# nv-tlabs/DefTet

Hardware: AMD Instinct MI355X
Metric: M tet-point tests/s (fwd+bwd) at res=70, 100k queries (higher is better)
Workload: dtype f32

## Files before the change

deftet_amd/csrc/point_in_tet.hip:

```cpp
#pragma clang fp contract(off)

#include <stdlib.h>

#include <algorithm>
#include <type_traits>
#include <vector>

#include "common.hpp"

namespace deftet {
namespace pit {

constexpr float kBig = 1048576.0f;
constexpr float kTau = 1.0f / 128.0f;
constexpr float kMargin = 1.0f / 64.0f;
constexpr float kWMin = 9.3132257e-10f;
constexpr int kMiss = 0x7F7F7F7F;
constexpr int kMaxG = 112;
constexpr int kMaxBins = 15 * 1024;
constexpr int kHitOverflow = -2;

constexpr int kHitPad = 64;
__host__ __device__ inline int hit_pad(int B) { return (B + kHitPad - 1) / kHitPad * kHitPad; }
__host__ __device__ inline size_t hit_cnt_off(int B, int T) { return (size_t)B * T * 2; }
// ... 1225 lines not shown
            if (__builtin_amdgcn_ballot_w64(cnew > cap) != 0ull) {
                if (cnew > cap) {
                    int *resb = result + (size_t)b * Q;
                    if (hcnt > 0) atomicMin(&resb[h0], t);
                    if (hcnt > 1) atomicMin(&resb[h1], t);
                    if (hcnt > 2) atomicMin(&resb[h2], t);
                    if (hcnt > 3) atomicMin(&resb[h3], t);
                    on_full();
                }
            }
#pragma unroll
            for (int k = 0; k < PIT_BATCH; ++k) {
                const int qi = __float_as_int(q[k].w);
                h3 = sel(acc[k], h2, h3);
                h2 = sel(acc[k], h1, h2);
                h1 = sel(acc[k], h0, h1);
                h0 = sel(acc[k], qi, h0);
                hcnt += sel(acc[k], 1, 0);
            }
            c += PIT_BATCH;
        }
    }
    PHASE_MARK(1);
    if (npend > 0) {
        const typename TS::Ref tv = ts.at(b, T, t);
        atomicAdd(&counters[gridDim.y * 4 + b * 4 + 1], npend);
        if (npend > 2) {
            exact_rescan<TS>(tv, t, tb, sq, result + (size_t)b * Q, G, Gx, cx0, cx1, cy0, cy1, cz0, cz1, m, counters, gridDim.y, b, hits, spill, (size_t)b * T + t);
            irregular_tail<TS>(tet, t, b, T, Q, pts, counters, irregQ, result);
            return;
        }
        for (int k = 0; k < npend; ++k) {
            const float4 q = sq[k == 0 ? pend0 : pend1];
            if (exact_accept<TS>(tv, q.x, q.y, q.z) > 0.f) {
                const int qi = __float_as_int(q.w);
                atomicMin(&result[(size_t)b * Q + qi], t);
                if (hcnt >= cap) {
                    int *resb = result + (size_t)b * Q;
                    atomicMin(&resb[h0], t); atomicMin(&resb[h1], t);
                    if (hcnt > 2) atomicMin(&resb[h2], t);
                    if (hcnt > 3) atomicMin(&resb[h3], t);
                    on_full();
                }
                h3 = h2; h2 = h1; h1 = h0; h0 = qi;
                ++hcnt;
            }
        }
    }
    int *resb = uniform_ptr(result + (size_t)b * Q);
    if (hcnt > 0) atomic_smin_off(resb, (unsigned)h0 * 4u, t);
    if (hcnt > 1) atomic_smin_off(resb, (unsigned)h1 * 4u, t);
    if (hcnt > 2) atomic_smin_off(resb, (unsigned)h2 * 4u, t);
    if (hcnt > 3) atomic_smin_off(resb, (unsigned)h3 * 4u, t);
    if (full == 1 && hcnt > cap) full = 2;
    if (full == 2) note_overflow(counters, gridDim.y, b, t);
    if (hits) {
        if (full == 0) {
            const lanemask_t sp = mask_of(hcnt > 2);
            store_b64_off(uniform_ptr(hits + (size_t)b * T), (unsigned)t * 8u, sel(sp, h0 | kHitSpilled, h0), h1);
            if (hcnt > 2) store_b128_off(uniform_ptr(spill + (size_t)b * T), (unsigned)t * 16u, h2, h3, -1, -1);
        } else if (full == 1) {
            int *sp = reinterpret_cast<int *>(spill + (size_t)b * T + t) + scnt;
            if (hcnt > 0) sp[0] = h0;
            if (hcnt > 1) sp[1] = h1;
            if (hcnt > 2) sp[2] = h2;
            if (hcnt > 3) sp[3] = h3;
        } else {
            store_b64_off(uniform_ptr(hits + (size_t)b * T), (unsigned)t * 8u, -1, kHitOverflow);
        }
    }
    irregular_tail<TS>(tet, t, b, T, Q, pts, counters, irregQ, result);
    PHASE_MARK(2);
}

constexpr int kWvRows = 192;
#ifndef PIT_WVCAP
#define PIT_WVCAP 96
#endif
constexpr int kWvCap = PIT_WVCAP;
constexpr int kWvSlots = 6;
#ifndef PIT_WG
#define PIT_WG 128
#endif
constexpr int kWvThreads = PIT_WG;
static_assert(kWvThreads % 64 == 0 && kWvThreads >= 64 && kWvThreads <= 256, "whole waves");
static_assert(kWvRows % 64 == 0 && kWvSlots >= 4 && kWvSlots <= 8, "whole waves of row ids; the records hold four + four");
#ifndef PIT_WVCAP_PAIR
#define PIT_WVCAP_PAIR 128
#endif
constexpr int kWvCapPair = PIT_WVCAP_PAIR, kWvRowsPair = 256;
#ifndef PIT_DBG_WALK
#define PIT_DBG_WALK 1
#endif
#ifndef PIT_DBG_PEND
#define PIT_DBG_PEND 1
#endif
#ifndef PIT_STOP
#define PIT_STOP 0
#endif
#define PIT_KEEP(x) asm volatile("" ::"v"(x))
#ifndef PIT_PROBE_SKIP
#define PIT_PROBE_SKIP 0
#endif
#ifndef PIT_PROBE_PREFILL
#define PIT_PROBE_PREFILL 0
#endif
#ifndef PIT_PIN_SHAPES
#define PIT_PIN_SHAPES 0
#endif
#ifndef PIT_PROBE_SCATTER
#define PIT_PROBE_SCATTER 0
#endif
#ifndef PIT_WAVES_PAIR
#define PIT_WAVES_PAIR 5
#endif
#ifndef PIT_TOLX
#define PIT_TOLX 2
#endif
#ifndef PIT_MINGROUP
#define PIT_MINGROUP 4
#endif
constexpr int kWvMinGroup = PIT_MINGROUP;
#ifndef PIT_ZREACH
#define PIT_ZREACH 24
#endif
constexpr int kWvZReach = PIT_ZREACH;
constexpr float kRelScale = 2.86102294921875e-06f;
constexpr float kTauSlim = kTau * (1.0f + 1.0f / 128.0f);
#ifndef PIT_WAVES2
#define PIT_WAVES2 7
#endif
template <int CAP, int ROWS>
struct __attribute__((aligned(16))) WaveStageT {
    typedef typename std::conditional<(ROWS <= 254), unsigned char, unsigned short>::type marker_t;
    float4 q[CAP];
    int delta[ROWS];
    unsigned short rowBase[ROWS + 4];
    marker_t marker[CAP];
};

template <int CTRL, int ROW_MASK>
__device__ __forceinline__ int dpp0(int v)
{
    return __builtin_amdgcn_update_dpp(0, v, CTRL, ROW_MASK, 0xf, true);
}
__device__ __forceinline__ int wave_scan_add(int x)
{
    x += dpp0<0x111, 0xf>(x); x += dpp0<0x112, 0xf>(x); x += dpp0<0x114, 0xf>(x); x += dpp0<0x118, 0xf>(x);
    x += dpp0<0x142, 0xa>(x); x += dpp0<0x143, 0xc>(x);
    return x;
}
__device__ __forceinline__ int wave_scan_max(int x)
{
    x = max(x, dpp0<0x111, 0xf>(x)); x = max(x, dpp0<0x112, 0xf>(x)); x = max(x, dpp0<0x114, 0xf>(x)); x = max(x, dpp0<0x118, 0xf>(x));
    x = max(x, dpp0<0x142, 0xa>(x)); x = max(x, dpp0<0x143, 0xc>(x));
    return x;
}
typedef unsigned short u16x2 __attribute__((ext_vector_type(2)));
__device__ __forceinline__ unsigned pk_max(unsigned a, unsigned b)
{
    const u16x2 r = __builtin_elementwise_max(__builtin_bit_cast(u16x2, a), __builtin_bit_cast(u16x2, b));
    return __builtin_bit_cast(unsigned, r);
}
__device__ __forceinline__ unsigned wave_pk_max(unsigned v)
{
    v = pk_max(v, (unsigned)dpp0<0x111, 0xf>((int)v)); v = pk_max(v, (unsigned)dpp0<0x112, 0xf>((int)v));
    v = pk_max(v, (unsigned)dpp0<0x114, 0xf>((int)v)); v = pk_max(v, (unsigned)dpp0<0x118, 0xf>((int)v));
    v = pk_max(v, (unsigned)dpp0<0x142, 0xf>((int)v)); v = pk_max(v, (unsigned)dpp0<0x143, 0xf>((int)v));
    return (unsigned)__builtin_amdgcn_readlane((int)v, 63);
}
__device__ __forceinline__ void wave_sync()
{
    __builtin_amdgcn_fence(__ATOMIC_ACQ_REL, "wavefront");
    __builtin_amdgcn_wave_barrier();
}
__device__ __forceinline__ void atomic_smin_off_nh(int *base, unsigned byte_off, int v)
{
    asm volatile("global_atomic_smin %0, %1, %2" ::"v"(byte_off), "v"(v), "s"(base) : "memory");
}

__device__ __forceinline__ float sel(lanemask_t m, float if_set, float if_clear)
{
    return __int_as_float(sel(m, __float_as_int(if_set), __float_as_int(if_clear)));
}
__device__ __forceinline__ void cross_fma(float ax, float ay, float az, float bx, float by, float bz, float *n)
{
    n[0] = fmaf(ay, bz, -(az * by));
    n[1] = fmaf(az, bx, -(ax * bz));
    n[2] = fmaf(ax, by, -(ay * bx));
}

template <class TS>
__device__ __noinline__ void irregular_tet_slow(typename TS::Arg tet, int t, int b, int T, int Q, const float *__restrict__ pts,
                                                int *counters, int *irregT, const int *__restrict__ irregQ, int *result, int2 *hits)
{
    const int k = atomicAdd(&counters[b * 4 + 0], 1);
    irregT[(size_t)b * T + k] = t;
    if (hits) hits[(size_t)b * T + t] = make_int2(-1, kHitOverflow);
    if (counters[b * 4 + 1] > 0) irregular_tail_slow<TS>(tet, t, b, T, Q, pts, counters, irregQ, result);
}

__device__ __forceinline__ void tet_cell_box(const float *__restrict__ tv, const Grid &g, int G, int Gx, CellBox &cb, float &mrg)
{
    float blo[3], bhi[3], wk[3];
#pragma unroll
    for (int k = 0; k < 3; ++k) {
        blo[k] = fminf(fminf(tv[k], tv[3 + k]), fminf(tv[6 + k], tv[9 + k]));
        bhi[k] = fmaxf(fmaxf(tv[k], tv[3 + k]), fmaxf(tv[6 + k], tv[9 + k]));
        wk[k] = bhi[k] - blo[k];
    }
    const float w = fmaxf(fmaxf(wk[0], wk[1]), wk[2]);
    mrg = w * kMargin;
    cb.cx0 = cell_of(blo[0] - mrg, g.o[0], g.inv[0], Gx); cb.cx1 = cell_of(bhi[0] + mrg, g.o[0], g.inv[0], Gx);
    cb.cy0 = cell_of(blo[1] - mrg, g.o[1], g.inv[1], G); cb.cy1 = cell_of(bhi[1] + mrg, g.o[1], g.inv[1], G);
    cb.cz0 = cell_of(blo[2] - mrg, g.o[2], g.inv[2], G); cb.cz1 = cell_of(bhi[2] + mrg, g.o[2], g.inv[2], G);
}

template <class TS>
__device__ __noinline__ int exact_rescan_slots(typename TS::RefArg tv, int t, const int *__restrict__ tb, const float4 *__restrict__ sq,
                                               int *res, const float *__restrict__ gp, int G, int Gx, int *slotCol)
{
    float vv[12];
    TS::get(tv, vv);
    Planes P;
    make_planes(vv, P);
    const Grid g = load_grid(gp);
    CellBox cb;
    float m;
    tet_cell_box(vv, g, G, Gx, cb, m);
    float elo[3], ehi[3];
#pragma unroll
    for (int k = 0; k < 3; ++k) {
        elo[k] = fminf(fminf(vv[k], vv[3 + k]), fminf(vv[6 + k], vv[9 + k])) - m;
        ehi[k] = fmaxf(fmaxf(vv[k], vv[3 + k]), fmaxf(vv[6 + k], vv[9 + k])) + m;
    }
    const int Gp = table_pitch(G);
    int hcnt = 0;
    for (int cz = cb.cz0; cz <= cb.cz1; ++cz)
        for (int cy = cb.cy0; cy <= cb.cy1; ++cy) {
            const int s = tb[table_off(cz, cb.cx0, cy, Gx, Gp)], e = tb[table_off(cz, cb.cx1 + 1, cy, Gx, Gp)];
            for (int j = s; j < e; ++j) {
                const float4 q = sq[j];
                if (q.x >= elo[0] && q.x <= ehi[0] && q.y >= elo[1] && q.y <= ehi[1] && q.z >= elo[2] && q.z <= ehi[2] &&
                    accept(P, q.x, q.y, q.z)) {
                    const int qi = __float_as_int(q.w);
                    atomicMin(&res[qi], t);
                    slotCol[min(hcnt, kWvSlots) * kWvThreads] = qi;
                    ++hcnt;
                }
            }
        }
    return hcnt;
}

__device__ __forceinline__ float triple(const float *a, const float *b, const float *c)
{
    float x0 = b[1] * c[2] - b[2] * c[1];
    float x1 = b[2] * c[0] - b[0] * c[2];
    float x2 = b[0] * c[1] - b[1] * c[0];
    return (a[0] * x0 + a[1] * x1) + a[2] * x2;
}
__device__ __forceinline__ float4 bary_weights(const float4 t0, const float4 t1, const float4 t2, float px, float py, float pz)
{
    const float A[3] = {t0.x, t0.y, t0.z}, Bv[3] = {t0.w, t1.x, t1.y}, Cv[3] = {t1.z, t1.w, t2.x}, D[3] = {t2.y, t2.z, t2.w};
    const float pp[3] = {px, py, pz};
    float vap[3], vbp[3], vab[3], vac[3], vad[3], vbc[3], vbd[3];
#pragma unroll
    for (int k = 0; k < 3; ++k) {
        vap[k] = pp[k] - A[k]; vbp[k] = pp[k] - Bv[k];
        vab[k] = Bv[k] - A[k]; vac[k] = Cv[k] - A[k]; vad[k] = D[k] - A[k];
        vbc[k] = Cv[k] - Bv[k]; vbd[k] = D[k] - Bv[k];
    }
    const float v6 = 1.0f / triple(vab, vac, vad);
    float4 wq;
    wq.x = triple(vbp, vbd, vbc) * v6;
    wq.y = triple(vap, vac, vad) * v6;
    wq.z = triple(vap, vad, vab) * v6;
    wq.w = triple(vap, vab, vac) * v6;
    return wq;
}

template <class TS, bool ORD, int NT>
__device__ __forceinline__ void tet_scan_wave_body(typename TS::Arg tet, int T, int Q,
                                                  const float *__restrict__ gparam, int G, int Gx, const int *__restrict__ table,
                                                  long long cellStride, const float4 *__restrict__ sortedQ, int *result, int *counters,
                                                  int *irregT, int2 *hits, const float *__restrict__ pts,
                                                  const int *__restrict__ irregQ, int *ucount, int hpad, int4 *spill,
                                                  const int *__restrict__ order)
{
    constexpr int CAP = NT == 1 ? kWvCap : kWvCapPair, ROWS = NT == 1 ? kWvRows : kWvRowsPair;
    typedef WaveStageT<CAP, ROWS> Stage;
    __shared__ Stage s_w[kWvThreads / 64];
    __shared__ int s_hit[NT][kWvSlots + 2][kWvThreads];
#if PIT_PIN_SHAPES
    const int pinL = blockIdx.y * gridDim.x + blockIdx.x, pinB = gridDim.y;
#define PIT_BLK_B (pinL % pinB)
#define PIT_BLK_X (pinL / pinB)
#else
#define PIT_BLK_B blockIdx.y
#define PIT_BLK_X blockIdx.x
#endif
    if (ucount && PIT_BLK_X == 0 && __builtin_amdgcn_readfirstlane(threadIdx.x) == 0) {
        ucount[PIT_BLK_B] = 0;
        ucount[hpad + PIT_BLK_B] = 0;
        ucount[2 * hpad + PIT_BLK_B] = 0;
    }
    const int b = PIT_BLK_B, tid = threadIdx.x, lane = tid & 63;
    const TS ts(tet);
    Stage &W = s_w[tid >> 6];
    const int nblk = gridDim.x;
#if PIT_PIN_SHAPES
    const int vb = PIT_BLK_X;
#else
    const int per = (nblk + 7) >> 3;
    const int vb = (blockIdx.x & 7) * per + (blockIdx.x >> 3);
#endif
#undef PIT_BLK_B
#undef PIT_BLK_X
    const int t = vb * blockDim.x + tid;
    const bool valid = vb < nblk && t < (T + NT - 1) / NT;
    if (__builtin_amdgcn_ballot_w64(valid) == 0ull) return;
    auto tet_id = [&](int k) -> int {
        const int p = min(NT * t + k, T - 1);
        return ORD ? order[p] : p;
    };
    auto tet_exists = [&](int k) -> bool { return valid && (NT == 1 || NT * t + k < T); };
    PHASE_DECL;
    SPAN_MARK(0);
    const Grid g = load_grid(gparam + b * kGridWords);
    Filter F[NT];
    float eabsMax[NT], mrg[NT], wk[NT][3];
    bool regular[NT], works[NT];
    int cx0 = 0x7FFF, cx1 = 0, cy0 = 0x7FFF, cy1 = 0, cz0 = 0x7FFF, cz1 = 0;
#pragma unroll
    for (int k = 0; k < NT; ++k) {
        float v[12];
        TS::template get4<PIT_SCAN_TET_NT != 0>(ts.at(b, T, tet_id(k)), v);
        float mN[4][3], det;
        {
            const float e1x = v[3] - v[0], e1y = v[4] - v[1], e1z = v[5] - v[2];
            const float e2x = v[6] - v[0], e2y = v[7] - v[1], e2z = v[8] - v[2];
            const float e3x = v[9] - v[0], e3y = v[10] - v[1], e3z = v[11] - v[2];
            cross_fma(e1x, e1y, e1z, e2x, e2y, e2z, mN[0]);
            cross_fma(e3x, e3y, e3z, e1x, e1y, e1z, mN[1]);
            cross_fma(e2x, e2y, e2z, e3x, e3y, e3z, mN[2]);
#pragma unroll
            for (int j = 0; j < 3; ++j) mN[3][j] = -((mN[0][j] + mN[1][j]) + mN[2][j]);
            det = fmaf(mN[0][0], e3x, fmaf(mN[0][1], e3y, mN[0][2] * e3z));
        }
        float blo[3], bhi[3], mx[3];
#pragma unroll
        for (int j = 0; j < 3; ++j) {
            blo[j] = fminf(fminf(v[j], v[3 + j]), fminf(v[6 + j], v[9 + j]));
            bhi[j] = fmaxf(fmaxf(v[j], v[3 + j]), fmaxf(v[6 + j], v[9 + j]));
            wk[k][j] = bhi[j] - blo[j];
            mx[j] = fmaxf(fabsf(blo[j]), fabsf(bhi[j]));
        }
        const float w = fmaxf(fmaxf(wk[k][0], wk[k][1]), wk[k][2]);
        regular[k] = fmaxf(fmaxf(mx[0], mx[1]), mx[2]) <= kBig && w >= kWMin && fabsf(det) >= kTauSlim * ((w * w) * w);
        mrg[k] = w * kMargin;
        float elo[3], ehi[3];
#pragma unroll
        for (int j = 0; j < 3; ++j) {
            elo[j] = blo[j] - mrg[k];
            ehi[j] = bhi[j] + mrg[k];
        }
        const bool ingrid = !(ehi[0] < g.lo[0] || elo[0] > g.hi[0] || ehi[1] < g.lo[1] || elo[1] > g.hi[1] || ehi[2] < g.lo[2] || elo[2] > g.hi[2]);
        {
            const int ax0 = cell_of(elo[0], g.o[0], g.inv[0], Gx), ax1 = cell_of(ehi[0], g.o[0], g.inv[0], Gx);
            const int ay0 = cell_of(elo[1], g.o[1], g.inv[1], G), ay1 = cell_of(ehi[1], g.o[1], g.inv[1], G);
            const int az0 = cell_of(elo[2], g.o[2], g.inv[2], G), az1 = cell_of(ehi[2], g.o[2], g.inv[2], G);
            regular[k] = regular[k] && !(ingrid && wide_tet(ax0, ax1, ay0, ay1, az0, az1, g));
            works[k] = tet_exists(k) && regular[k] && ingrid;
            if (NT == 1) {
                cx0 = ax0; cx1 = ax1; cy0 = ay0; cy1 = ay1; cz0 = az0; cz1 = az1;
            } else if (works[k]) {
                cx0 = min(cx0, ax0); cx1 = max(cx1, ax1); cy0 = min(cy0, ay0); cy1 = max(cy1, ay1); cz0 = min(cz0, az0); cz1 = max(cz1, az1);
            }
        }
        const float sigma = det > 0.f ? 1.0f : -1.0f;
        float S[3];
#pragma unroll
        for (int j = 0; j < 3; ++j) S[j] = fmaf(mx[j], 2.0f * kErrScale, g.pe[j]);
        eabsMax[k] = 0.f;
#pragma unroll
        for (int i = 0; i < 4; ++i) {
            const float n0 = mN[i][0], n1 = mN[i][1], n2 = mN[i][2];
            const float *a = i < 3 ? v : v + 3;
            const float c = fmaf(n0, a[0], fmaf(n1, a[1], n2 * a[2]));
            const float E = fmaf(fabsf(n0), S[0], fmaf(fabsf(n1), S[1], fabsf(n2) * S[2]));
            F[k].N[i][0] = sigma * n0; F[k].N[i][1] = sigma * n1; F[k].N[i][2] = sigma * n2;
            F[k].C[i] = fmaf(-sigma, c, -E);
            eabsMax[k] = fmaxf(eabsMax[k], E);
        }
    }
    bool work = works[0];
#pragma unroll
    for (int k = 1; k < NT; ++k) work = work || works[k];
    if (PIT_STOP == 1) {
#pragma unroll
        for (int i = 0; i < 4; ++i) { PIT_KEEP(F[0].N[i][0]); PIT_KEEP(F[0].N[i][1]); PIT_KEEP(F[0].N[i][2]); PIT_KEEP(F[0].C[i]); }
        PIT_KEEP(eabsMax[0]); PIT_KEEP(mrg[0]); PIT_KEEP(wk[0][0]); PIT_KEEP(wk[0][1]); PIT_KEEP(wk[0][2]);
        PIT_KEEP(cx0); PIT_KEEP(cx1); PIT_KEEP(cy0); PIT_KEEP(cy1); PIT_KEEP(cz0); PIT_KEEP(cz1); PIT_KEEP((int)work);
        return;
    }
    const int Gp = table_pitch(G);
    const int *tb = table + (size_t)b * cellStride;
    const float4 *sq = sortedQ + (size_t)b * Q;
    int gx0[2], gx1[2], gy0[2], gz0[2], gny[2], gnz[2], gsh[2];
    int gid = -1;
    int ncx = cx1 - cx0 + 1, ncy = cy1 - cy0 + 1;
    int rowsTot = 0, rowOff1 = 0, slabsTot = 0;
    {
        lanemask_t rem = __builtin_amdgcn_ballot_w64(work);
        int ng = 0;
#pragma unroll
        for (int p = 0; p < 2; ++p) {
            gx0[p] = gx1[p] = gy0[p] = gz0[p] = 0;
            gny[p] = gnz[p] = gsh[p] = 0;
        }
#pragma unroll
        for (int p = 0; p < 3; ++p) {
            if (ng == 2 || __popcll(rem) < kWvMinGroup) break;
            const int pl = __ffsll((long long)rem) - 1;
            const int px0 = __builtin_amdgcn_readlane(cx0, pl), px1 = __builtin_amdgcn_readlane(cx1, pl);
            const int py0 = __builtin_amdgcn_readlane(cy0, pl), py1 = __builtin_amdgcn_readlane(cy1, pl);
            const int pz0 = __builtin_amdgcn_readlane(cz0, pl);
            const bool in = ((rem >> lane) & 1ull) != 0ull && (unsigned)(cx0 - px0 + PIT_TOLX) <= 2u * PIT_TOLX && (unsigned)(cx1 - px1 + PIT_TOLX) <= 2u * PIT_TOLX &&
                            (unsigned)(cy0 - py0 + 1) <= 2u && (unsigned)(cy1 - py1 + 1) <= 2u && (unsigned)(cz0 - pz0 + kWvZReach) <= 2u * kWvZReach;
            const lanemask_t gm = __builtin_amdgcn_ballot_w64(in);
            rem &= ~gm;
            if (__popcll(gm) < kWvMinGroup) { REASON_COUNT(2, gm); continue; }
            const unsigned ax = wave_pk_max(in ? ((unsigned)cx1 | ((0xFFFFu - (unsigned)cx0) << 16)) : 0u);
            const unsigned ay = wave_pk_max(in ? ((unsigned)cy1 | ((0xFFFFu - (unsigned)cy0) << 16)) : 0u);
            const unsigned az = wave_pk_max(in ? ((unsigned)cz1 | ((0xFFFFu - (unsigned)cz0) << 16)) : 0u);
            const int ux0 = (int)(0xFFFFu - (ax >> 16)), uy0 = (int)(0xFFFFu - (ay >> 16)), uz0 = (int)(0xFFFFu - (az >> 16));
            const int ny = (int)(ay & 0xFFFFu) - uy0 + 1, nz = (int)(az & 0xFFFFu) - uz0 + 1;
            const int sh = ny <= 1 ? 0 : 32 - __builtin_clz((unsigned)(ny - 1));
            if (sh > 2 || slabsTot + nz > 64 || rowsTot + (nz << sh) > ROWS) {
                REASON_COUNT(sh > 2 ? 3 : slabsTot + nz > 64 ? 4 : 5, gm);
                continue;
            }
            const bool second = ng != 0;
            gx0[0] = second ? gx0[0] : ux0; gx1[0] = second ? gx1[0] : (int)(ax & 0xFFFFu); gy0[0] = second ? gy0[0] : uy0; gz0[0] = second ? gz0[0] : uz0;
            gny[0] = second ? gny[0] : ny; gnz[0] = second ? gnz[0] : nz; gsh[0] = second ? gsh[0] : sh;
            gx0[1] = second ? ux0 : 0; gx1[1] = second ? (int)(ax & 0xFFFFu) : 0; gy0[1] = second ? uy0 : 0; gz0[1] = second ? uz0 : 0;
            gny[1] = second ? ny : 0; gnz[1] = second ? nz : 0; gsh[1] = second ? sh : 0;
            if (second) rowOff1 = rowsTot;
            rowsTot += nz << sh;
            slabsTot += nz;
            if (in) { gid = ng; ncx = (int)(ax & 0xFFFFu) - ux0 + 1; ncy = ny; }
            ++ng;
        }
        REASON_COUNT(6, rem);
    }
#pragma unroll
    for (int k = 0; k < NT; ++k) {
        const float R0 = fmaf(2.0f, mrg[k], wk[k][0]) + (float)(ncx + 1) * g.cs[0];
        const float R1 = fmaf(2.0f, mrg[k], wk[k][1]) + (float)(ncy + 1) * g.cs[1];
        const float R2 = fmaf(2.0f, mrg[k], wk[k][2]) + (float)(cz1 - cz0 + 2) * g.cs[2];
        const float erel = fmaf(kRelScale, fmaf(wk[k][1] * wk[k][2], R0, fmaf(wk[k][0] * wk[k][2], R1, (wk[k][0] * wk[k][1]) * R2)), kErrAbs);
#pragma unroll
        for (int i = 0; i < 4; ++i) F[k].C[i] -= erel;
        F[k].twoEmax = 2.0f * (eabsMax[k] + erel);
        if (NT > 1 && !works[k]) {
#pragma unroll
            for (int i = 0; i < 4; ++i) { F[k].N[i][0] = F[k].N[i][1] = F[k].N[i][2] = 0.f; F[k].C[i] = -INFINITY; }
            F[k].twoEmax = 0.f;
        }
    }
    if (PIT_STOP == 2) {
#pragma unroll
        for (int i = 0; i < 4; ++i) { PIT_KEEP(F[0].N[i][0]); PIT_KEEP(F[0].N[i][1]); PIT_KEEP(F[0].N[i][2]); PIT_KEEP(F[0].C[i]); }
        PIT_KEEP(F[0].twoEmax); PIT_KEEP(gid); PIT_KEEP(rowsTot); PIT_KEEP(rowOff1); PIT_KEEP(cz0); PIT_KEEP(cz1);
        return;
    }
    PHASE_MARK(0);
    int *resb = uniform_ptr(result + (size_t)b * Q);
    asm volatile("s_nop 4" ::: "memory");
    unsigned slot0[NT], slotEnd[NT], slotA[NT];
#pragma unroll
    for (int k = 0; k < NT; ++k) {
        slot0[k] = (unsigned)(k * (kWvSlots + 2) * kWvThreads + tid) * 4u;
        slotEnd[k] = slot0[k] + (unsigned)(kWvSlots + 1) * (unsigned)(kWvThreads * 4);
        slotA[k] = slot0[k];
    }
    int pend0 = -1, pend1 = -1, npend = 0;
    typedef float f32x2 __attribute__((ext_vector_type(2)));
    f32x2 Px01[NT], Py01[NT], Pz01[NT], Pc01[NT], Px23[NT], Py23[NT], Pz23[NT], Pc23[NT];
#pragma unroll
    for (int k = 0; k < NT; ++k) {
        Px01[k] = f32x2{F[k].N[0][0], F[k].N[1][0]}; Py01[k] = f32x2{F[k].N[0][1], F[k].N[1][1]};
        Pz01[k] = f32x2{F[k].N[0][2], F[k].N[1][2]}; Pc01[k] = f32x2{F[k].C[0], F[k].C[1]};
        Px23[k] = f32x2{F[k].N[2][0], F[k].N[3][0]}; Py23[k] = f32x2{F[k].N[2][1], F[k].N[3][1]};
        Pz23[k] = f32x2{F[k].N[2][2], F[k].N[3][2]}; Pc23[k] = f32x2{F[k].C[2], F[k].C[3]};
    }
    auto test = [&](const float4 q) {
        const f32x2 qx = {q.x, q.x}, qy = {q.y, q.y}, qz = {q.z, q.z};
        const int qi = __float_as_int(q.w);
        float av[NT];
#pragma unroll
        for (int k = 0; k < NT; ++k) {
            const f32x2 A01 = __builtin_elementwise_fma(Px01[k], qx, __builtin_elementwise_fma(Py01[k], qy, __builtin_elementwise_fma(Pz01[k], qz, Pc01[k])));
            const f32x2 A23 = __builtin_elementwise_fma(Px23[k], qx, __builtin_elementwise_fma(Py23[k], qy, __builtin_elementwise_fma(Pz23[k], qz, Pc23[k])));
            av[k] = fminf(fminf(A01.x, A01.y), fminf(A23.x, A23.y));
        }
#pragma unroll
        for (int k = 0; k < NT; ++k)
            if (av[k] > F[k].twoEmax) {
                *reinterpret_cast<int *>(reinterpret_cast<char *>(&s_hit[0][0][0]) + slotA[k]) = qi;
                slotA[k] = min(slotA[k] + (unsigned)(kWvThreads * 4), slotEnd[k]);
            }
        bool band = fabsf(av[0]) <= F[0].twoEmax;
#pragma unroll
        for (int k = 1; k < NT; ++k) band = band || fabsf(av[k]) <= F[k].twoEmax;
        if (__builtin_amdgcn_ballot_w64(band) != 0ull) {
            asm volatile("" ::: "memory");
#pragma unroll
            for (int k = 0; k < NT; ++k) {
                const bool bk = fabsf(av[k]) <= F[k].twoEmax;
                pend1 = bk ? pend0 : pend1;
                pend0 = bk ? (qi | (k << 30)) : pend0;
                npend = bk ? npend + 1 : npend;
            }
        }
    };
    if (rowsTot > 0) {
        const int nzA = gnz[0];
        const bool second = lane >= nzA, slabLane = lane < slabsTot;
        const lanemask_t m2 = mask_of(second);
        const int zl = sel(m2, lane - nzA, lane), sh = sel(m2, gsh[1], gsh[0]), ny = sel(m2, gny[1], gny[0]);
        const int rowId0 = sel(m2, rowOff1, 0) + (zl << sh);
        int a[4], len[4];
        {
            const unsigned zrow = (unsigned)(sel(m2, gz0[1], gz0[0]) + (slabLane ? zl : 0)) * (unsigned)(Gx + 1);
            const unsigned la = ((zrow + (unsigned)sel(m2, gx0[1], gx0[0])) * (unsigned)Gp + (unsigned)sel(m2, gy0[1], gy0[0])) * 4u;
            const unsigned le = ((zrow + (unsigned)sel(m2, gx1[1], gx1[0]) + 1u) * (unsigned)Gp + (unsigned)sel(m2, gy0[1], gy0[0])) * 4u;
            const int4u a0 = ld_off_u4(tb, la), e0 = ld_off_u4(tb, le);
            a[0] = a0.x; a[1] = a0.y; a[2] = a0.z; a[3] = a0.w;
            len[0] = e0.x - a0.x; len[1] = e0.y - a0.y; len[2] = e0.z - a0.z; len[3] = e0.w - a0.w;
        }
        int pre[5];
        pre[0] = 0;
        int lmax = 0;
#pragma unroll
        for (int y = 0; y < 4; ++y) {
            len[y] = sel(mask_of(slabLane && y < ny), len[y], 0);
            pre[y + 1] = pre[y] + len[y];
            lmax = max(lmax, len[y]);
        }
        const int incl = wave_scan_add(pre[4]);
        const int lb = incl - pre[4];
        const int N = __builtin_amdgcn_readlane(incl, 63);
        const int Rtot = rowsTot;
        const bool fitsRows = __builtin_amdgcn_ballot_w64(lmax > CAP) == 0ull && N < 65536;
        if (slabLane) {
#pragma unroll
            for (int y = 0; y < 4; ++y)
                if (y < (1 << sh)) {
                    W.rowBase[rowId0 + y] = (unsigned short)(lb + pre[y]);
                    W.delta[rowId0 + y] = a[y] - (lb + pre[y]);
                }
        }
        if (lane == 0) W.rowBase[Rtot] = (unsigned short)N;
        wave_sync();
        if (PIT_STOP == 3) {
#pragma unroll
            for (int i = 0; i < 4; ++i) { PIT_KEEP(F[0].N[i][0]); PIT_KEEP(F[0].N[i][1]); PIT_KEEP(F[0].N[i][2]); PIT_KEEP(F[0].C[i]); }
            PIT_KEEP(F[0].twoEmax); PIT_KEEP(gid); PIT_KEEP(N); PIT_KEEP(lb); PIT_KEEP(cz0); PIT_KEEP(cz1);
            return;
        }
        PHASE_MARK(4);
        const lanemask_t mine2 = mask_of(gid == 1);
        const int rowOff = sel(mine2, rowOff1, 0), gz = sel(mine2, gz0[1], gz0[0]), gs = sel(mine2, gsh[1], gsh[0]);
        int rn = rowOff + ((cz0 - gz) << gs);
        const int re = rowOff + ((cz1 + 1 - gz) << gs);
        if (!fitsRows) { REASON_COUNT(7, __builtin_amdgcn_ballot_w64(gid >= 0)); gid = -1; }
        int r0 = fitsRows ? 0 : Rtot;
#pragma unroll 1
        while (r0 < Rtot) {
            const int B0 = __builtin_amdgcn_readfirstlane(W.rowBase[r0]);
            int r1 = Rtot;
            if (N - B0 > CAP) {
                r1 = r0;
#pragma unroll 1
                for (int j = 0; j < ROWS / 64; ++j) {
                    const int rc = r0 + 1 + lane + 64 * j;
                    const int cnt = rc <= Rtot ? W.rowBase[rc] - B0 : 0x7FFFFFFF;
                    const lanemask_t fits = __builtin_amdgcn_ballot_w64(cnt <= CAP);
                    if (fits == ~0ull) { r1 += 64; continue; }
                    r1 += __ffsll((long long)~fits) - 1;
                    break;
                }
            }
            const int Nc = __builtin_amdgcn_readfirstlane(W.rowBase[r1]) - B0;
            for (int i = lane; i < Nc; i += 64) W.marker[i] = 0;
            wave_sync();
            if (slabLane) {
                int p0 = W.rowBase[rowId0];
#pragma unroll
                for (int y = 0; y < 4; ++y) {
                    if (y < (1 << sh)) {
                        const int r = rowId0 + y, p1 = W.rowBase[r + 1];
                        if (p1 > p0 && r >= r0 && r < r1) W.marker[p0 - B0] = (typename Stage::marker_t)(r + 1);
                        p0 = p1;
                    }
                }
            }
            wave_sync();
            int carry = 0;
#pragma unroll
            for (int j = 0; j < (CAP + 63) / 64; ++j)
                if (j * 64 < Nc) {
                    const int i = lane + 64 * j;
                    const int own = max(wave_scan_max(i < Nc ? W.marker[i] : 0), carry);
                    carry = __builtin_amdgcn_readlane(own, 63);
                    if (i < Nc) W.q[i] = ld_off<float4>(sq, (unsigned)(B0 + i + W.delta[own - 1]) * 16u);
                }
            wave_sync();
            PHASE_MARK(5);
            PHASE_COUNT(7, Nc);
            PHASE_COUNT(15, 1);
            const int lo = max(rn, r0), hi = min(re, r1);
            if (PIT_STOP != 4 && gid >= 0 && lo < hi) {
                unsigned c = (unsigned)(W.rowBase[lo] - B0) * 16u;
                const unsigned e = (unsigned)(W.rowBase[hi] - B0) * 16u;
                PHASE_COUNT(13, (e - c) >> 4);
                rn = hi;
                const char *qb0 = reinterpret_cast<const char *>(&W.q[0]);
                if (c < e) {
                    float4 qa = *reinterpret_cast<const float4 *>(qb0 + c);
                    for (;;) {
                        const float4 qb = *reinterpret_cast<const float4 *>(qb0 + c + 16);
                        test(qa);
                        c += 16;
                        if (c >= e) break;
                        qa = *reinterpret_cast<const float4 *>(qb0 + c + 16);
                        test(qb);
                        c += 16;
                        if (c >= e) break;
                    }
                }
            }
            wave_sync();
            PHASE_MARK(6);
            r0 = r1;
        }
    }
    PHASE_COUNT(14, __popcll(__builtin_amdgcn_ballot_w64(work && gid < 0)));
    PHASE_MARK(1);
    if (PIT_DBG_WALK && work && gid < 0) {
        CellBox cb;
        {
            cb.cx0 = cb.cy0 = cb.cz0 = 0x7FFF;
            cb.cx1 = cb.cy1 = cb.cz1 = 0;
#pragma unroll
            for (int k = 0; k < NT; ++k) {
                if (NT > 1 && !works[k]) continue;
                float tv[12], mrg2;
                TS::get(ts.at(b, T, tet_id(k)), tv);
                CellBox c1;
                tet_cell_box(tv, g, G, Gx, c1, mrg2);
                cb.cx0 = min(cb.cx0, c1.cx0); cb.cx1 = max(cb.cx1, c1.cx1); cb.cy0 = min(cb.cy0, c1.cy0); cb.cy1 = max(cb.cy1, c1.cy1);
                cb.cz0 = min(cb.cz0, c1.cz0); cb.cz1 = max(cb.cz1, c1.cz1);
            }
        }
        const int cx0 = cb.cx0, cx1 = cb.cx1, cy0 = cb.cy0, cy1 = cb.cy1, cz1 = cb.cz1, czn = cb.cz0;
        const int ny = cy1 - cy0 + 1;
        const unsigned lineB = (unsigned)Gp * 4u;
        const unsigned slabB = (unsigned)(Gx + 1) * lineB;
        const unsigned dxB = (unsigned)(cx1 + 1 - cx0) * lineB;
        unsigned offS = ((unsigned)czn * (unsigned)(Gx + 1) + (unsigned)cx0) * lineB + (unsigned)cy0 * 4u;
        int cz = czn, yoff = 0;
        int4u nS = ld_off_u4(tb, offS), nE = ld_off_u4(tb, offS + dxB);
        bool haveNext = true;
        int c = 0, P1 = 0, P2 = 0, P3 = 0, P4 = 0, o0 = 0, o1 = 0, o2 = 0, o3 = 0;
        while (c < P4 || haveNext) {
            if (c >= P4) {
                const int rem = ny - yoff;
                const int n0 = nE.x - nS.x;
                const int n1 = rem > 1 ? nE.y - nS.y : 0;
                const int n2 = rem > 2 ? nE.z - nS.z : 0;
                const int n3 = rem > 3 ? nE.w - nS.w : 0;
                P1 = n0; P2 = P1 + n1; P3 = P2 + n2; P4 = P3 + n3;
                o0 = nS.x; o1 = nS.y - P1; o2 = nS.z - P2; o3 = nS.w - P3;
                c = 0;
                asm volatile("" : "+v"(P1), "+v"(P2), "+v"(P3), "+v"(P4), "+v"(o0), "+v"(o1), "+v"(o2), "+v"(o3));
                const bool wrap = rem <= 4;
                offS += wrap ? slabB - (unsigned)yoff * 4u : 16u;
                yoff = wrap ? 0 : yoff + 4;
                cz += wrap ? 1 : 0;
                haveNext = cz <= cz1;
                if (haveNext) {
                    nS = ld_off_u4(tb, offS);
                    nE = ld_off_u4(tb, offS + dxB);
                }
            }
            if (c < P4) {
                const int jq = c + (c < P1 ? o0 : c < P2 ? o1 : c < P3 ? o2 : o3);
                test(ld_off<float4>(sq, (unsigned)jq * 16u));
                ++c;
            }
        }
    }
    PHASE_MARK(2);
    if (PIT_STOP == 5) { PIT_KEEP(slotA[0]); PIT_KEEP(pend0); PIT_KEEP(pend1); PIT_KEEP(npend); return; }
    if (!valid) return;
    int hcnt[NT];
#pragma unroll
    for (int k = 0; k < NT; ++k) hcnt[k] = (int)((slotA[k] - slot0[k]) / (unsigned)(kWvThreads * 4));
    if (PIT_DBG_PEND && npend > 0) {
        atomicAdd(&counters[gridDim.y * 4 + b * 4 + 1], npend);
        if (npend > 2) {
#pragma unroll
            for (int k = 0; k < NT; ++k)
                if (works[k]) {
                    const int te = tet_id(k);
                    hcnt[k] = exact_rescan_slots<TS>(ts.at(b, T, te), te, tb, sq, result + (size_t)b * Q, gparam + b * kGridWords, G, Gx,
                                                 &s_hit[k][0][tid]);
                }
        } else {
            for (int j = 0; j < npend; ++j) {
                const int pq = j == 0 ? pend0 : pend1;
                const int k = NT == 1 ? 0 : (pq >> 30) & 1, qi = pq & 0x3FFFFFFF;
                const int te = tet_id(k);
                const float *pp = pts + ((size_t)b * Q + qi) * 3;
                if (exact_accept<TS>(ts.at(b, T, te), pp[0], pp[1], pp[2]) > 0.f) {
                    atomicMin(&result[(size_t)b * Q + qi], te);
                    if (NT == 1 || k == 0) { s_hit[0][min(hcnt[0], kWvSlots)][tid] = qi; ++hcnt[0]; }
                    else { s_hit[NT - 1][min(hcnt[NT - 1], kWvSlots)][tid] = qi; ++hcnt[NT - 1]; }
                }
            }
        }
    }
#pragma unroll
    for (int k = 0; k < NT; ++k) {
        if (NT > 1 && !tet_exists(k)) continue;
        int te = tet_id(k);
        asm volatile("" : "+v"(te));
        if (!regular[k]) {
            irregular_tet_slow<TS>(tet, te, b, T, Q, pts, counters, irregT, irregQ, result, hits);
            continue;
        }
        int hc = hcnt[k];
        if (hc > kWvSlots) {
            const typename TS::Ref tv = ts.at(b, T, te);
            hc = exact_rescan_slots<TS>(tv, te, tb, sq, result + (size_t)b * Q, gparam + b * kGridWords, G, Gx, &s_hit[k][0][tid]);
        }
#pragma unroll 1
        for (int i = 0; i < kWvSlots; ++i) {
            if (__builtin_amdgcn_ballot_w64(hc > i) == 0ull) break;
#if PIT_PROBE_SCATTER == 0
            if (hc > i && !(PIT_PROBE_SKIP & 1)) atomic_smin_off_nh(resb, (unsigned)s_hit[k][i][tid] * 4u, te);
#else
            if (hc > i && spill) {
                const int qi = s_hit[k][i][tid];
                char *pb = reinterpret_cast<char *>(spill);
                const size_t nq = (size_t)gridDim.y * Q, iq = (size_t)b * Q + qi;
                bool win = true;
                if (PIT_PROBE_SCATTER == 1) atomic_smin_off_nh(resb, (unsigned)qi * 4u, te);
                else win = atomicMin(&result[iq], te) > te;
                if (win && PIT_PROBE_SCATTER == 3) {
                    float4 s0, s1, s2;
                    TS::get3(ts.at(b, T, te), s0, s1, s2);
                    const float *pp = pts + iq * 3;
                    *reinterpret_cast<float4 *>(pb + iq * 16) = bary_weights(s0, s1, s2, pp[0], pp[1], pp[2]);
                    *reinterpret_cast<float *>(pb + nq * 16 + iq * 4) = (float)te;
                    *reinterpret_cast<float *>(pb + nq * 20 + iq * 4) = (float)qi;
                } else if (win) {
                    *reinterpret_cast<float4 *>(pb + iq * 16) = make_float4((float)te, (float)qi, 0.25f, 0.5f);
                    *reinterpret_cast<float *>(pb + nq * 16 + iq * 4) = (float)te;
                    *reinterpret_cast<float *>(pb + nq * 20 + iq * 4) = (float)qi;
                }
            }
#endif
        }
        if (hits) {
            int h[kRecSlots + kSpillSlots];
#pragma unroll
            for (int i = 0; i < kRecSlots + kSpillSlots; ++i) h[i] = -1;
#pragma unroll
            for (int i = 0; i < kRecSlots; ++i)
                if (i < hc) h[i] = s_hit[k][i][tid];
            const bool spilled = hc > kRecSlots && hc <= kWvSlots && spill != nullptr && PIT_PROBE_SCATTER == 0;
            const bool over = hc > kRecSlots && !spilled;
            if (spilled) {
#pragma unroll
                for (int i = kRecSlots; i < kWvSlots; ++i)
                    if (i < hc) h[i] = s_hit[k][i][tid];
                spill[(size_t)b * T + te] = make_int4(h[2], h[3], h[4], h[5]);
                h[0] |= kHitSpilled;
            }
            if (over) note_overflow(counters, gridDim.y, b, te);
            if (!(PIT_PROBE_SKIP & 2)) store_rec(hits + (size_t)b * T + te, over ? make_int2(-1, kHitOverflow) : make_int2(h[0], h[1]));
        }
        irregular_tail<TS>(tet, te, b, T, Q, pts, counters, irregQ, result);
    }
    PHASE_MARK(3);
    SPAN_MARK(1);
// ... 1298 lines not shown
```

Measured before the change: 1.102 billion.

## Pack per-tet setup into f32x2/u16x2 SIMD ops and simplify wave grouping

Vectorizes the per-tet filter setup (margins, cell coordinates, plane constants, sigma scaling) with packed f32x2 math, and replaces cell_of with a fmed3 clamp. Wave grouping now compares packed 16-bit x/y ranges and gets group bounds through ballots over tolerance offsets, which removes two packed max reductions. Slab address setup precomputes per-group bases, and the chunk loop tracks B0 incrementally with an unrolled marker clear. The goal is to cut VALU and cross-lane instruction count in setup. It carries a risk of subtle equivalence issues, for example the clamp semantics of cell_of versus fmed3.

Result: no change. 1.101 billion, median of 2 (-0.1%).

```diff
diff --git a/deftet_amd/csrc/point_in_tet.hip b/deftet_amd/csrc/point_in_tet.hip
--- a/deftet_amd/csrc/point_in_tet.hip
+++ b/deftet_amd/csrc/point_in_tet.hip
@@ -1401,9 +1401,10 @@
 }
 __device__ __forceinline__ int wave_scan_max(int x)
 {
-    x = max(x, dpp0<0x111, 0xf>(x)); x = max(x, dpp0<0x112, 0xf>(x)); x = max(x, dpp0<0x114, 0xf>(x)); x = max(x, dpp0<0x118, 0xf>(x));
-    x = max(x, dpp0<0x142, 0xa>(x)); x = max(x, dpp0<0x143, 0xc>(x));
-    return x;
+    unsigned u = (unsigned)x;
+    u = max(u, (unsigned)dpp0<0x111, 0xf>((int)u)); u = max(u, (unsigned)dpp0<0x112, 0xf>((int)u)); u = max(u, (unsigned)dpp0<0x114, 0xf>((int)u));
+    u = max(u, (unsigned)dpp0<0x118, 0xf>((int)u)); u = max(u, (unsigned)dpp0<0x142, 0xa>((int)u)); u = max(u, (unsigned)dpp0<0x143, 0xc>((int)u));
+    return (int)u;
 }
 typedef unsigned short u16x2 __attribute__((ext_vector_type(2)));
 __device__ __forceinline__ unsigned pk_max(unsigned a, unsigned b)
@@ -1577,6 +1578,7 @@
     PHASE_DECL;
     SPAN_MARK(0);
     const Grid g = load_grid(gparam + b * kGridWords);
+    typedef float f32x2 __attribute__((ext_vector_type(2)));
     Filter F[NT];
     float eabsMax[NT], mrg[NT], wk[NT][3];
     bool regular[NT], works[NT];
@@ -1609,16 +1611,20 @@
         regular[k] = fmaxf(fmaxf(mx[0], mx[1]), mx[2]) <= kBig && w >= kWMin && fabsf(det) >= kTauSlim * ((w * w) * w);
         mrg[k] = w * kMargin;
         float elo[3], ehi[3];
+        f32x2 cf[3];
 #pragma unroll
         for (int j = 0; j < 3; ++j) {
-            elo[j] = blo[j] - mrg[k];
-            ehi[j] = bhi[j] + mrg[k];
+            const f32x2 e = f32x2{blo[j], bhi[j]} + f32x2{-mrg[k], mrg[k]};
+            elo[j] = e.x;
+            ehi[j] = e.y;
+            cf[j] = (e - f32x2{g.o[j], g.o[j]}) * f32x2{g.inv[j], g.inv[j]};
         }
         const bool ingrid = !(ehi[0] < g.lo[0] || elo[0] > g.hi[0] || ehi[1] < g.lo[1] || elo[1] > g.hi[1] || ehi[2] < g.lo[2] || elo[2] > g.hi[2]);
         {
-            const int ax0 = cell_of(elo[0], g.o[0], g.inv[0], Gx), ax1 = cell_of(ehi[0], g.o[0], g.inv[0], Gx);
-            const int ay0 = cell_of(elo[1], g.o[1], g.inv[1], G), ay1 = cell_of(ehi[1], g.o[1], g.inv[1], G);
-            const int az0 = cell_of(elo[2], g.o[2], g.inv[2], G), az1 = cell_of(ehi[2], g.o[2], g.inv[2], G);
+            auto cell = [](float f, int n) -> int { return (int)__builtin_amdgcn_fmed3f(f, 0.f, (float)(n - 1)); };
+            const int ax0 = cell(cf[0].x, Gx), ax1 = cell(cf[0].y, Gx);
+            const int ay0 = cell(cf[1].x, G), ay1 = cell(cf[1].y, G);
+            const int az0 = cell(cf[2].x, G), az1 = cell(cf[2].y, G);
             regular[k] = regular[k] && !(ingrid && wide_tet(ax0, ax1, ay0, ay1, az0, az1, g));
             works[k] = tet_exists(k) && regular[k] && ingrid;
             if (NT == 1) {
@@ -1632,15 +1638,33 @@
 #pragma unroll
         for (int j = 0; j < 3; ++j) S[j] = fmaf(mx[j], 2.0f * kErrScale, g.pe[j]);
         eabsMax[k] = 0.f;
+        float cc[4], EE[4];
 #pragma unroll
         for (int i = 0; i < 4; ++i) {
             const float n0 = mN[i][0], n1 = mN[i][1], n2 = mN[i][2];
             const float *a = i < 3 ? v : v + 3;
-            const float c = fmaf(n0, a[0], fmaf(n1, a[1], n2 * a[2]));
-            const float E = fmaf(fabsf(n0), S[0], fmaf(fabsf(n1), S[1], fabsf(n2) * S[2]));
-            F[k].N[i][0] = sigma * n0; F[k].N[i][1] = sigma * n1; F[k].N[i][2] = sigma * n2;
-            F[k].C[i] = fmaf(-sigma, c, -E);
-            eabsMax[k] = fmaxf(eabsMax[k], E);
+            if (i >= 2) cc[i] = fmaf(n0, a[0], fmaf(n1, a[1], n2 * a[2]));
+            EE[i] = fmaf(fabsf(n0), S[0], fmaf(fabsf(n1), S[1], fabsf(n2) * S[2]));
+            eabsMax[k] = fmaxf(eabsMax[k], EE[i]);
+        }
+        {
+            const f32x2 c01 = __builtin_elementwise_fma(f32x2{mN[0][0], mN[1][0]}, f32x2{v[0], v[0]},
+                              __builtin_elementwise_fma(f32x2{mN[0][1], mN[1][1]}, f32x2{v[1], v[1]}, f32x2{mN[0][2], mN[1][2]} * f32x2{v[2], v[2]}));
+            cc[0] = c01.x;
+            cc[1] = c01.y;
+        }
+        const f32x2 sg = {sigma, sigma};
+#pragma unroll
+        for (int h = 0; h < 4; h += 2) {
+#pragma unroll
+            for (int j = 0; j < 3; ++j) {
+                const f32x2 n = sg * f32x2{mN[h][j], mN[h + 1][j]};
+                F[k].N[h][j] = n.x;
+                F[k].N[h + 1][j] = n.y;
+            }
+            const f32x2 C = __builtin_elementwise_fma(-sg, f32x2{cc[h], cc[h + 1]}, -f32x2{EE[h], EE[h + 1]});
+            F[k].C[h] = C.x;
+            F[k].C[h + 1] = C.y;
         }
     }
     bool work = works[0];
@@ -1663,6 +1687,8 @@
     {
         lanemask_t rem = __builtin_amdgcn_ballot_w64(work);
         int ng = 0;
+        const u16x2 xx = {(unsigned short)cx0, (unsigned short)cx1}, yy = {(unsigned short)cy0, (unsigned short)cy1};
+        const unsigned zz = (unsigned)cz1 | ((0xFFFFu - (unsigned)cz0) << 16);
 #pragma unroll
         for (int p = 0; p < 2; ++p) {
             gx0[p] = gx1[p] = gy0[p] = gz0[p] = 0;
@@ -1670,35 +1696,46 @@
         }
 #pragma unroll
         for (int p = 0; p < 3; ++p) {
-            if (ng == 2 || __popcll(rem) < kWvMinGroup) break;
+            if (ng == 2 || (int)__popcll(rem) < kWvMinGroup) break;
             const int pl = __ffsll((long long)rem) - 1;
-            const int px0 = __builtin_amdgcn_readlane(cx0, pl), px1 = __builtin_amdgcn_readlane(cx1, pl);
-            const int py0 = __builtin_amdgcn_readlane(cy0, pl), py1 = __builtin_amdgcn_readlane(cy1, pl);
+            const unsigned pxx = (unsigned)__builtin_amdgcn_readlane((int)__builtin_bit_cast(unsigned, xx), pl);
+            const unsigned pyy = (unsigned)__builtin_amdgcn_readlane((int)__builtin_bit_cast(unsigned, yy), pl);
             const int pz0 = __builtin_amdgcn_readlane(cz0, pl);
-            const bool in = ((rem >> lane) & 1ull) != 0ull && (unsigned)(cx0 - px0 + PIT_TOLX) <= 2u * PIT_TOLX && (unsigned)(cx1 - px1 + PIT_TOLX) <= 2u * PIT_TOLX &&
-                            (unsigned)(cy0 - py0 + 1) <= 2u && (unsigned)(cy1 - py1 + 1) <= 2u && (unsigned)(cz0 - pz0 + kWvZReach) <= 2u * kWvZReach;
-            const lanemask_t gm = __builtin_amdgcn_ballot_w64(in);
+            const int px0 = (int)(pxx & 0xFFFFu), px1 = (int)(pxx >> 16), py0 = (int)(pyy & 0xFFFFu), py1 = (int)(pyy >> 16);
+            const u16x2 bx = {(unsigned short)(px0 - PIT_TOLX), (unsigned short)(px1 - PIT_TOLX)}, by = {(unsigned short)(py0 - 1), (unsigned short)(py1 - 1)};
+            const u16x2 tolx = {2 * PIT_TOLX, 2 * PIT_TOLX}, toly = {2, 2};
+            const unsigned dx = __builtin_bit_cast(unsigned, (u16x2)(xx - bx)), dy = __builtin_bit_cast(unsigned, (u16x2)(yy - by));
+            const lanemask_t gm = __builtin_amdgcn_ballot_w64(pk_max(dx, __builtin_bit_cast(unsigned, tolx)) == __builtin_bit_cast(unsigned, tolx)) &
+                                  __builtin_amdgcn_ballot_w64(pk_max(dy, __builtin_bit_cast(unsigned, toly)) == __builtin_bit_cast(unsigned, toly)) &
+                                  __builtin_amdgcn_ballot_w64((unsigned)(cz0 - pz0 + kWvZReach) <= 2u * kWvZReach) & rem;
             rem &= ~gm;
-            if (__popcll(gm) < kWvMinGroup) { REASON_COUNT(2, gm); continue; }
-            const unsigned ax = wave_pk_max(in ? ((unsigned)cx1 | ((0xFFFFu - (unsigned)cx0) << 16)) : 0u);
-            const unsigned ay = wave_pk_max(in ? ((unsigned)cy1 | ((0xFFFFu - (unsigned)cy0) << 16)) : 0u);
-            const unsigned az = wave_pk_max(in ? ((unsigned)cz1 | ((0xFFFFu - (unsigned)cz0) << 16)) : 0u);
-            const int ux0 = (int)(0xFFFFu - (ax >> 16)), uy0 = (int)(0xFFFFu - (ay >> 16)), uz0 = (int)(0xFFFFu - (az >> 16));
-            const int ny = (int)(ay & 0xFFFFu) - uy0 + 1, nz = (int)(az & 0xFFFFu) - uz0 + 1;
+            if ((int)__popcll(gm) < kWvMinGroup) { REASON_COUNT(2, gm); continue; }
+            int lox = PIT_TOLX, hix = PIT_TOLX;
+#pragma unroll
+            for (int j = PIT_TOLX - 1; j >= 0; --j) {
+                lox = (__builtin_amdgcn_ballot_w64((unsigned short)dx <= (unsigned short)j) & gm) != 0ull ? j : lox;
+                hix = (__builtin_amdgcn_ballot_w64(dx >= ((unsigned)(2 * PIT_TOLX - j) << 16)) & gm) != 0ull ? 2 * PIT_TOLX - j : hix;
+            }
+            const int loy = (__builtin_amdgcn_ballot_w64((unsigned short)dy == 0) & gm) != 0ull ? 0 : 1;
+            const int hiy = (__builtin_amdgcn_ballot_w64(dy >= (2u << 16)) & gm) != 0ull ? 2 : 1;
+            const int ux0 = px0 - PIT_TOLX + lox, ux1 = px1 - PIT_TOLX + hix, uy0 = py0 - 1 + loy, uy1 = py1 - 1 + hiy;
+            const unsigned az = wave_pk_max(sel(gm, zz, 0u));
+            const int uz0 = (int)(0xFFFFu - (az >> 16));
+            const int ny = uy1 - uy0 + 1, nz = (int)(az & 0xFFFFu) - uz0 + 1;
             const int sh = ny <= 1 ? 0 : 32 - __builtin_clz((unsigned)(ny - 1));
             if (sh > 2 || slabsTot + nz > 64 || rowsTot + (nz << sh) > ROWS) {
                 REASON_COUNT(sh > 2 ? 3 : slabsTot + nz > 64 ? 4 : 5, gm);
                 continue;
             }
             const bool second = ng != 0;
-            gx0[0] = second ? gx0[0] : ux0; gx1[0] = second ? gx1[0] : (int)(ax & 0xFFFFu); gy0[0] = second ? gy0[0] : uy0; gz0[0] = second ? gz0[0] : uz0;
+            gx0[0] = second ? gx0[0] : ux0; gx1[0] = second ? gx1[0] : ux1; gy0[0] = second ? gy0[0] : uy0; gz0[0] = second ? gz0[0] : uz0;
             gny[0] = second ? gny[0] : ny; gnz[0] = second ? gnz[0] : nz; gsh[0] = second ? gsh[0] : sh;
-            gx0[1] = second ? ux0 : 0; gx1[1] = second ? (int)(ax & 0xFFFFu) : 0; gy0[1] = second ? uy0 : 0; gz0[1] = second ? uz0 : 0;
+            gx0[1] = second ? ux0 : 0; gx1[1] = second ? ux1 : 0; gy0[1] = second ? uy0 : 0; gz0[1] = second ? uz0 : 0;
             gny[1] = second ? ny : 0; gnz[1] = second ? nz : 0; gsh[1] = second ? sh : 0;
             if (second) rowOff1 = rowsTot;
             rowsTot += nz << sh;
             slabsTot += nz;
-            if (in) { gid = ng; ncx = (int)(ax & 0xFFFFu) - ux0 + 1; ncy = ny; }
+            gid = sel(gm, ng, gid); ncx = sel(gm, ux1 - ux0 + 1, ncx); ncy = sel(gm, ny, ncy);
             ++ng;
         }
         REASON_COUNT(6, rem);
@@ -1710,7 +1747,11 @@
         const float R2 = fmaf(2.0f, mrg[k], wk[k][2]) + (float)(cz1 - cz0 + 2) * g.cs[2];
         const float erel = fmaf(kRelScale, fmaf(wk[k][1] * wk[k][2], R0, fmaf(wk[k][0] * wk[k][2], R1, (wk[k][0] * wk[k][1]) * R2)), kErrAbs);
 #pragma unroll
-        for (int i = 0; i < 4; ++i) F[k].C[i] -= erel;
+        for (int i = 0; i < 4; i += 2) {
+            const f32x2 C = f32x2{F[k].C[i], F[k].C[i + 1]} - f32x2{erel, erel};
+            F[k].C[i] = C.x;
+            F[k].C[i + 1] = C.y;
+        }
         F[k].twoEmax = 2.0f * (eabsMax[k] + erel);
         if (NT > 1 && !works[k]) {
 #pragma unroll
@@ -1735,7 +1776,6 @@
         slotA[k] = slot0[k];
     }
     int pend0 = -1, pend1 = -1, npend = 0;
-    typedef float f32x2 __attribute__((ext_vector_type(2)));
     f32x2 Px01[NT], Py01[NT], Pz01[NT], Pc01[NT], Px23[NT], Py23[NT], Pz23[NT], Pc23[NT];
 #pragma unroll
     for (int k = 0; k < NT; ++k) {
@@ -1776,15 +1816,23 @@
     };
     if (rowsTot > 0) {
         const int nzA = gnz[0];
-        const bool second = lane >= nzA, slabLane = lane < slabsTot;
-        const lanemask_t m2 = mask_of(second);
-        const int zl = sel(m2, lane - nzA, lane), sh = sel(m2, gsh[1], gsh[0]), ny = sel(m2, gny[1], gny[0]);
-        const int rowId0 = sel(m2, rowOff1, 0) + (zl << sh);
+        const bool slabLane = lane < slabsTot;
+        const int lc = min(lane, slabsTot - 1);
+        const lanemask_t mS = mask_of(slabLane), m2 = mask_of(lc >= nzA);
+        const unsigned slabB = (unsigned)(Gx + 1) * (unsigned)Gp * 4u;
+        unsigned bA[2], bE[2];
+#pragma unroll
+        for (int p = 0; p < 2; ++p) {
+            const unsigned zrow = (unsigned)gz0[p] * (unsigned)(Gx + 1) - (p ? (unsigned)nzA * (unsigned)(Gx + 1) : 0u);
+            bA[p] = ((zrow + (unsigned)gx0[p]) * (unsigned)Gp + (unsigned)gy0[p]) * 4u;
+            bE[p] = ((zrow + (unsigned)gx1[p] + 1u) * (unsigned)Gp + (unsigned)gy0[p]) * 4u;
+        }
+        const int pitch = sel(m2, 1 << gsh[1], 1 << gsh[0]);
+        const int rowId0 = sel(m2, rowOff1 + ((lc - nzA) << gsh[1]), lc << gsh[0]);
         int a[4], len[4];
         {
-            const unsigned zrow = (unsigned)(sel(m2, gz0[1], gz0[0]) + (slabLane ? zl : 0)) * (unsigned)(Gx + 1);
-            const unsigned la = ((zrow + (unsigned)sel(m2, gx0[1], gx0[0])) * (unsigned)Gp + (unsigned)sel(m2, gy0[1], gy0[0])) * 4u;
-            const unsigned le = ((zrow + (unsigned)sel(m2, gx1[1], gx1[0]) + 1u) * (unsigned)Gp + (unsigned)sel(m2, gy0[1], gy0[0])) * 4u;
+            const unsigned lz = __umul24((unsigned)lc, slabB);
+            const unsigned la = lz + sel(m2, bA[1], bA[0]), le = lz + sel(m2, bE[1], bE[0]);
             const int4u a0 = ld_off_u4(tb, la), e0 = ld_off_u4(tb, le);
             a[0] = a0.x; a[1] = a0.y; a[2] = a0.z; a[3] = a0.w;
             len[0] = e0.x - a0.x; len[1] = e0.y - a0.y; len[2] = e0.z - a0.z; len[3] = e0.w - a0.w;
@@ -1794,7 +1842,8 @@
         int lmax = 0;
 #pragma unroll
         for (int y = 0; y < 4; ++y) {
-            len[y] = sel(mask_of(slabLane && y < ny), len[y], 0);
+            const lanemask_t my = y == 0 ? mS : mS & ((y < gny[1] ? m2 : 0ull) | (y < gny[0] ? ~m2 : 0ull));
+            len[y] = sel(my, len[y], 0);
             pre[y + 1] = pre[y] + len[y];
             lmax = max(lmax, len[y]);
         }
@@ -1806,7 +1855,7 @@
         if (slabLane) {
 #pragma unroll
             for (int y = 0; y < 4; ++y)
-                if (y < (1 << sh)) {
+                if (y < pitch) {
                     W.rowBase[rowId0 + y] = (unsigned short)(lb + pre[y]);
                     W.delta[rowId0 + y] = a[y] - (lb + pre[y]);
                 }
@@ -1826,11 +1875,11 @@
         const int re = rowOff + ((cz1 + 1 - gz) << gs);
         if (!fitsRows) { REASON_COUNT(7, __builtin_amdgcn_ballot_w64(gid >= 0)); gid = -1; }
         int r0 = fitsRows ? 0 : Rtot;
+        int B0 = 0;
 #pragma unroll 1
         while (r0 < Rtot) {
-            const int B0 = __builtin_amdgcn_readfirstlane(W.rowBase[r0]);
-            int r1 = Rtot;
-            if (N - B0 > CAP) {
+            int r1 = Rtot, Nc = N - B0;
+            if (Nc > CAP) {
                 r1 = r0;
 #pragma unroll 1
                 for (int j = 0; j < ROWS / 64; ++j) {
@@ -1841,15 +1890,20 @@
                     r1 += __ffsll((long long)~fits) - 1;
                     break;
                 }
-            }
-            const int Nc = __builtin_amdgcn_readfirstlane(W.rowBase[r1]) - B0;
-            for (int i = lane; i < Nc; i += 64) W.marker[i] = 0;
+                Nc = __builtin_amdgcn_readfirstlane(W.rowBase[r1]) - B0;
+            }
+#pragma unroll
+            for (int j = 0; j < (CAP + 63) / 64; ++j)
+                if (j * 64 < Nc) {
+                    const int i = lane + 64 * j;
+                    if (i < Nc) W.marker[i] = 0;
+                }
             wave_sync();
             if (slabLane) {
                 int p0 = W.rowBase[rowId0];
 #pragma unroll
                 for (int y = 0; y < 4; ++y) {
-                    if (y < (1 << sh)) {
+                    if (y < pitch) {
                         const int r = rowId0 + y, p1 = W.rowBase[r + 1];
                         if (p1 > p0 && r >= r0 && r < r1) W.marker[p0 - B0] = (typename Stage::marker_t)(r + 1);
                         p0 = p1;
@@ -1894,6 +1948,7 @@
             wave_sync();
             PHASE_MARK(6);
             r0 = r1;
+            B0 += Nc;
         }
     }
     PHASE_COUNT(14, __popcll(__builtin_amdgcn_ballot_w64(work && gid < 0)));
```
